# theblackcat102/edgedict

Hardware: AMD Instinct MI355X
Metric: utterances/sec (E6D2, 15 s audio) (higher is better)
Workload: dtype bf16; 1 GPU; E6D2 full training step (dither+log-mel+stack3+SpecAugment masks -> 6x1024 LSTM encoder, 2x time reduction -> 2x256 LSTM prediction net -> joint 640 -> RNN-T loss -> backward -> grad all-reduce -> Adam); 64 x 15 s utterances per GPU, U=64, V=2048, ragged lengths; lattice [64,201,65,2048]; global_batch=64, parallelism=dp1

## Files before the change

edgedict_amd/csrc/encoder_stack.hip:

```cpp
#include <stdio.h>
#include <stdlib.h>

#include <algorithm>
#include <mutex>
#include <vector>

#include "stack_kernels.hpp"

int ed_gemm_quiet_partials(int dtype_in, const void* A, long long lda, int a_kmajor, const void* B,
                           long long ldb, int b_kmajor, int M, int N, int K, int split_k,
                           int max_wg_per_cu, float* partials, int* slices, hipStream_t stream);

namespace {

__device__ __forceinline__ uint4 pack8(const float* v) {
    uint4 o;
    o.x = (unsigned)f32_to_bf16(v[0]) | ((unsigned)f32_to_bf16(v[1]) << 16);
    o.y = (unsigned)f32_to_bf16(v[2]) | ((unsigned)f32_to_bf16(v[3]) << 16);
    o.z = (unsigned)f32_to_bf16(v[4]) | ((unsigned)f32_to_bf16(v[5]) << 16);
    o.w = (unsigned)f32_to_bf16(v[6]) | ((unsigned)f32_to_bf16(v[7]) << 16);
    return o;
}
__device__ __forceinline__ int row_of_kap(int kap, int H) { return ((kap >> 4) & 3) * H + (kap >> 6) * 16 + (kap & 15); }

__global__ void pack_wih_kernel(const float* __restrict__ W, const float* __restrict__ b_ih,
                                const float* __restrict__ b_hh, bf16_t* __restrict__ Wp,
                                bf16_t* __restrict__ Wt, float* __restrict__ bp, int H, int I) {
    const long long n = 4ll * H * I;
    for (long long i = (long long)blockIdx.x * blockDim.x + threadIdx.x; i < n;
         i += (long long)gridDim.x * blockDim.x) {
        const int row = (int)(i / I), k = (int)(i % I);
        const int g = row / H, j = row % H;
        const int kap = ed_gate_col(g, j);
        const bf16_t v = f32_to_bf16(W[i]);
        Wp[(long long)kap * I + k] = v;
        if (Wt) Wt[(long long)k * 4 * H + kap] = v;
        if (k == 0) bp[kap] = b_ih[row] + b_hh[row];
    }
}
// ... 94 lines not shown
    for (long long c = (long long)blockIdx.x * blockDim.x + threadIdx.x; c < n4; c += (long long)gridDim.x * blockDim.x) {
        const int row = (int)(c / K4), k = (int)(c % K4) * 4;
        const long long o = (long long)ed_gate_col(row / H, row % H) * K + k;
        float4 v = make_float4(0.f, 0.f, 0.f, 0.f);
        for (int sl = 0; sl < S; ++sl) {
            const float4 p = *reinterpret_cast<const float4*>(src + sl * slice_stride + o);
            v.x += p.x; v.y += p.y; v.z += p.z; v.w += p.w;
        }
        const long long i = (long long)row * K + k;
        if (accumulate) {
            const float4 d = *reinterpret_cast<const float4*>(dst + i);
            *reinterpret_cast<float4*>(dst + i) = make_float4(d.x + v.x, d.y + v.y, d.z + v.z, d.w + v.w);
            if (dst2) {
                const float4 e = *reinterpret_cast<const float4*>(dst2 + i);
                *reinterpret_cast<float4*>(dst2 + i) = make_float4(e.x + v.x, e.y + v.y, e.z + v.z, e.w + v.w);
            }
        } else {
            *reinterpret_cast<float4*>(dst + i) = v;
            if (dst2) *reinterpret_cast<float4*>(dst2 + i) = v;
        }
    }
}
int unpermute_rows(const float* src, long long slice_stride, int S, float* dst, float* dst2, int H, int K, int accumulate,
                   hipStream_t s) {
    const bool vec = K % 4 == 0 && slice_stride % 4 == 0 && (uintptr_t)src % 16 == 0 && (uintptr_t)dst % 16 == 0 &&
                     (uintptr_t)dst2 % 16 == 0;
    if (vec)
        hipLaunchKernelGGL(unpermute_rows4_kernel, dim3(ed_grid_for(4ll * H * K / 4, 256, 4096)), dim3(256), 0, s, src,
                           slice_stride, S, dst, dst2, H, K, accumulate);
    else
        hipLaunchKernelGGL(unpermute_rows_kernel, dim3(ed_grid_for(4ll * H * K, 256, 4096)), dim3(256), 0, s, src,
                           slice_stride, S, dst, dst2, H, K, accumulate);
    ED_CHECK_LAUNCH("unpermute_rows_kernel");
    return ED_OK;
}

struct Runtime {
    std::mutex mu;
    hipStream_t R = nullptr, W = nullptr;
    int prio_hi = 0;
    hipEvent_t tev[2][2] = {{nullptr, nullptr}, {nullptr, nullptr}};
    int tlaunches[2] = {0, 0};
    int tkind[2] = {0, 0}, tsteps[2] = {0, 0};
    bool time_each = false;
    static constexpr int STAMP_SLOTS = 4096;
    unsigned long long* stamps[2] = {nullptr, nullptr};
    int stamp_used[2] = {0, 0};
    unsigned long long* stamp_slot(int i, hipStream_t s) {
        if (!time_each) return nullptr;
        if (!stamps[i] && hipMalloc((void**)&stamps[i], (size_t)STAMP_SLOTS * 16) != hipSuccess) {
            stamps[i] = nullptr;
            return nullptr;
        }
        if (stamp_used[i] == 0) {
            if (hipMemsetAsync(stamps[i], 0, (size_t)STAMP_SLOTS * 16, s) != hipSuccess) return nullptr;
            if (hipMemset2DAsync(stamps[i], 16, 0xff, 8, STAMP_SLOTS, s) != hipSuccess) return nullptr;
        }
        if (stamp_used[i] >= STAMP_SLOTS) return nullptr;
        return stamps[i] + 2 * (size_t)stamp_used[i]++;
    }
    unsigned* wsr_err_host = nullptr;
    unsigned* wsr_err_dev = nullptr;
    hipStream_t lazy(hipStream_t& s) {
        if (!s && hipStreamCreateWithPriority(&s, hipStreamNonBlocking, prio_hi) != hipSuccess) s = nullptr;
        return s;
    }
// ... 136 lines not shown
    for (int l = 0; l < d->L; ++l) {
        const edgedict_stack_layer_t& y = d->layers[l];
        ED_CHECK_ARG(y.T == T && y.I == I, "encoder_stack: layer %d geometry (T=%d I=%d) does not follow from the layers above (T=%d I=%d)", l, y.T, y.I, T, I);
        ED_CHECK_ARG(!y.residual || y.I == d->H, "encoder_stack: layer %d: residual needs I == H", l);
        ED_CHECK_ARG(y.drop_p >= 0.f && y.drop_p < 1.f, "encoder_stack: layer %d: dropout probability must be in [0, 1)", l);
        ED_CHECK_ARG(y.wih_p && y.bias_p && y.whh_f && y.ln_gamma && y.ln_beta && y.X && y.G && y.Yx && y.Cx && y.mean && y.rstd, "encoder_stack: layer %d: null pointer", l);
        if (backward)
            ED_CHECK_ARG(y.whh_b && y.dZ && (l == 0 || y.dX) && y.dW_ih && y.dW_hh && y.db && y.dgamma && y.dbeta, "encoder_stack: layer %d: null backward pointer", l);
        g[l].m = g[0].f / g[l].f;
        g[l].cf = d->chunk * g[l].f;
        g[l].nchunks = (y.T + g[l].cf - 1) / g[l].cf;
        T = (T + y.reduce - 1) / y.reduce;
        I = d->H;
    }
    ED_CHECK_ARG(d->ws_bytes >= ws_layout(d).total, "encoder_stack: workspace too small");
    return ED_OK;
}

struct Pace {
    static bool allows(int w, int l, int m_l, int m_min_running) {
        const int period = max(1, m_l / max(1, m_min_running));
        return period <= 1 || ((w + period * 1024 - (l % period)) % period) == 0;
    }
};

int margin_launches(const edgedict_stack_desc_t* d, const std::vector<Geom>& g, bool backward) {
    const int P = d->chunk * g[0].f;
    if (d->lag > 0) return max(1, d->lag - P + (backward ? 1 : 0));
    static const int mf = [] { const char* e = getenv("EDGEDICT_STACK_MARGIN_F"); return e ? atoi(e) : 0; }();
    static const int mb = [] { const char* e = getenv("EDGEDICT_STACK_MARGIN_B"); return e ? atoi(e) : 0; }();
    if (backward ? mb > 0 : mf > 0) return backward ? mb : mf;
    return backward ? 6 : 3;
}

#define ED_TRY(expr)            \
    do {                        \
        int st__ = (expr);      \
        if (st__ != ED_OK) return st__; \
    } while (0)

struct ScheduleTrace {
    int32_t* step_launch = nullptr;
    int32_t* chunk_enqueued = nullptr;
    std::vector<int> toff, coff;
    int launches = 0, max_slots = 0;
};
thread_local ScheduleTrace* g_trace = nullptr;
#define ED_DEV(expr)                      \
    do {                                  \
        if (!g_trace) ED_TRY(expr);       \
    } while (0)

struct Streams {
    hipStream_t C, R, R2, W;
    int split;
    int which(int l) const { return l >= split ? 1 : 0; }
    hipStream_t RS(int l) const { return which(l) ? R2 : R; }
    hipStream_t S[ED_STACK_MAX_SLOTS];
    bool serial;
    Runtime* rt;
    std::unique_lock<std::mutex> lock;
    hipEvent_t shared_ev = nullptr;
    hipStream_t shared_src = nullptr;
    int share(hipStream_t src) {
        if (serial) return ED_OK;
        shared_ev = rt->get();
        ED_CHECK_ARG(shared_ev != nullptr, "encoder_stack: event creation failed");
        ED_CHECK_HIP(hipEventRecord(shared_ev, src));
        shared_src = src;
        return ED_OK;
    }
    void unshare() { shared_ev = nullptr; shared_src = nullptr; }
// ... 717 lines not shown
                 "stack_launch_times: nothing recorded (edgedict_stack_time_launches(1) first)");
    const int n = r->stamp_used[i];
    std::vector<unsigned long long> h(2 * (size_t)n);
    ED_CHECK_HIP(hipStreamSynchronize(r->R));
    ED_CHECK_HIP(hipMemcpy(h.data(), r->stamps[i], h.size() * sizeof(unsigned long long), hipMemcpyDeviceToHost));
    double ticks = 0.0;
    int ok = 0;
    for (int k = 0; k < n; ++k)
        if (h[2 * k + 1] > h[2 * k]) {
            ticks += (double)(h[2 * k + 1] - h[2 * k]);
            ++ok;
        }
    ED_CHECK_ARG(ok > 0, "stack_launch_times: no launch stamped");
    *sum_ms = (float)(ticks * 1e-5);
    *launches = ok;
    return ED_OK;
}

extern "C" int edgedict_stack_launch_stamps(int backward, unsigned long long* out, int max_launches, int* launches) {
    ED_CHECK_ARG(out && launches && max_launches > 0, "stack_launch_stamps: bad arguments");
    Runtime* r = runtime_for_current_device();
    std::unique_lock<std::mutex> lock;
    if (r) lock = std::unique_lock<std::mutex>(r->mu);
    const int i = backward ? 1 : 0;
    ED_CHECK_ARG(r && r->stamps[i] && r->stamp_used[i] > 0,
                 "stack_launch_stamps: nothing recorded (edgedict_stack_time_launches(1) first)");
    const int n = min(max_launches, r->stamp_used[i]);
    ED_CHECK_HIP(hipDeviceSynchronize());
    ED_CHECK_HIP(hipMemcpy(out, r->stamps[i], (size_t)n * 16, hipMemcpyDeviceToHost));
    *launches = n;
    return ED_OK;
}

extern "C" int edgedict_stack_backward(const edgedict_stack_desc_t* d, void* stream_) {
    std::vector<Geom> g;
    ED_TRY(validate(d, g, true));
    ED_CHECK_ARG(d->dout && d->d_in_gamma && d->d_in_beta, "encoder_stack: null backward pointer in descriptor");
    ED_CHECK_ARG(!(d->flags & EDGEDICT_STACK_INFERENCE), "encoder_stack: backward on a descriptor flagged EDGEDICT_STACK_INFERENCE");
    const int B = d->B, H = d->H, L = d->L;
    const long long BH = (long long)B * H;
    const WsLayout wl = ws_layout(d);
    char* ws = (char*)d->ws;
    Streams st;
    ED_TRY(open_streams(d, stream_, st));
    st.R2 = st.R;
    st.split = L;
    const int T_out = (g[L - 1].T + d->layers[L - 1].reduce - 1) / d->layers[L - 1].reduce;

    static const int soft_env = [] { const char* e = getenv("EDGEDICT_STACK_SOFT_WAIT"); return e ? atoi(e) : 1; }();
    const bool soft = soft_env && !st.serial && L <= 8;
    unsigned* bflag = reinterpret_cast<unsigned*>(ws + wl.wsr_sync) + SYNC_BFLAG;
    unsigned* gerr = (st.rt && st.rt->wsr_err_dev) ? st.rt->wsr_err_dev + 2 : nullptr;
    if (soft)
        for (int l = 0; l < L; ++l) ED_CHECK_ARG(g[l].nchunks <= 512, "encoder_stack: too many chunks for the flag table");
    const int sk_ns = sk_bwd_steps(d);
    if (st.rt) {
        st.rt->tkind[1] = sk_ns ? 2 : 0;
        st.rt->tsteps[1] = sk_ns;
    }
    unsigned* cntb = reinterpret_cast<unsigned*>(ws + wl.wsr_sync) + SYNC_BCNT;
    unsigned* gcnt = reinterpret_cast<unsigned*>(ws + wl.wsr_sync) + SYNC_GCNT;
    if (sk_ns) {
        if (poison_on())
            for (int l = 0; l < L; ++l) {
                ED_DEV(ed_stack_fill(ws + wl.gimg[l], 0xff, (size_t)(d->layers[l].T + 1) * wl.gimg_stride, st.C));
                ED_DEV(ed_stack_fill(ws + wl.skpart[l], 0xff, (size_t)2 * (H / 64) * 4 * 64 * 64 * sizeof(float), st.C));
// ... 8 lines not shown
    ED_TRY(st.chain(st.C, st.W));

    std::vector<std::vector<hipEvent_t>> Eb(L);
    std::vector<std::vector<char>> queued(L);
    for (int l = 0; l < L; ++l) {
        Eb[l].assign(g[l].nchunks, nullptr);
        queued[l].assign(g[l].nchunks, l == L - 1 ? 1 : 0);
    }
    {
        const edgedict_stack_layer_t& y = d->layers[L - 1];
        hipStream_t S = st.S[L - 1];
        const DropCfg dcT = drop_of(y);
        for (int k = g[L - 1].nchunks - 1; k >= 0; --k) {
            const int t0 = k * g[L - 1].cf, t1 = min(y.T, t0 + g[L - 1].cf);
            ED_DEV(ed_stack_ln_bwd(bptr(d->dout), H, (long long)T_out * H, bptr(y.Yx) + BH,
                                   y.residual ? bptr(y.X) : nullptr, y.ln_gamma, y.mean, y.rstd, bptr(y.dZ),
                                   (float*)(ws + wl.lnpart[L - 1]) + (size_t)k * LNB_GRID * 2 * H, LNB_GRID, B, H,
                                   t0, t1, y.reduce, S, dcT.thresh, dcT.seed, dcT.scale, dcT.T_out));
            if (soft) ED_DEV(ed_stack_set_flag(bflag + (L - 1) * 512 + k, S));
            else ED_TRY(st.record(Eb[L - 1][k], S));
        }
    }
    std::vector<int> deferred;

    const int acc_grads = (d->flags & EDGEDICT_STACK_ACCUM_GRADS) ? 1 : 0;
    auto weight_grads = [&](int l, int t0, int t1, bool first, bool last_of_all) -> int {
        if (g_trace) {
            if (t0 == 0 && d->grads_final) d->grads_final(l, d->grads_final_user);
            return ED_OK;
        }
        const edgedict_stack_layer_t& y = d->layers[l];
        const int M = (t1 - t0) * B;
        const long long r0 = (long long)t0 * B;
        float* tmpW = (float*)(ws + wl.tmpW);
        float* tmpB = (float*)(ws + wl.tmpB);
        const int sk = d->split_k > 0 ? d->split_k : (last_of_all ? 8 : 2);
        const int cap = last_of_all ? 4 : 2;
        const int acc = (acc_grads || !first) ? 1 : 0;
        int S = 1;
        ED_TRY(ed_gemm_quiet_partials(ED_BF16, bptr(y.G) + r0 * 4 * H, 4ll * H, 0, bptr(y.X) + r0 * y.I, y.I, 0,
                                      4 * H, y.I, M, sk, cap, tmpW, &S, st.W));
        ED_TRY(unpermute_rows(tmpW, 4ll * H * y.I, S, y.dW_ih, nullptr, H, y.I, acc, st.W));
        ED_TRY(ed_gemm_quiet_partials(ED_BF16, bptr(y.G) + r0 * 4 * H, 4ll * H, 0, bptr(y.Yx) + r0 * H, H, 0,
                                      4 * H, H, M, sk, cap, tmpW, &S, st.W));
        ED_TRY(unpermute_rows(tmpW, 4ll * H * H, S, y.dW_hh, nullptr, H, H, acc, st.W));
        ED_TRY(ed_stack_zero(tmpB, (size_t)4 * H * sizeof(float), st.W));
        ED_TRY(edgedict_colsum(ED_BF16, bptr(y.G) + r0 * 4 * H, 4ll * H, tmpB, M, 4 * H, st.W));
        hipLaunchKernelGGL(unpermute_rows_kernel, dim3(ed_grid_for(4ll * H, 256, 4096)), dim3(256),
                           0, st.W, tmpB, 0, 1, y.db, y.db_hh, H, 1, acc);
        ED_CHECK_LAUNCH("unpermute_rows_kernel");
        if (t0 == 0 && d->grads_final) d->grads_final(l, d->grads_final_user);
        return ED_OK;
    };
    int dw_seg = 1 << 20;
    if (const char* e = getenv("EDGEDICT_STACK_DW_SEG")) dw_seg = max(1, atoi(e));
    if (d->flags & EDGEDICT_STACK_DW_AT_END) dw_seg = 1 << 20;
    int tail_split = 0;
    if (const char* e = getenv("EDGEDICT_STACK_TAIL_SPLIT")) tail_split = atoi(e);

    int margin = margin_launches(d, g, true);
    std::vector<int> next_t(L, 0);
    std::vector<std::vector<int>> ready_w(L);
    for (int l = 0; l < L; ++l) ready_w[l].assign(g[l].nchunks, l == L - 1 ? 0 : 0x3fffffff);
    auto after_recurrence = [&](int l, hipStream_t waiter) -> int { return st.chain(st.RS(l), waiter); };
    auto chunk_done = [&](int l, int k, int w) -> int {
            const edgedict_stack_layer_t& y = d->layers[l];
            if (l > 0) {
                const edgedict_stack_layer_t& z = d->layers[l - 1];
                const int t0 = k * g[l].cf, t1 = min(y.T, t0 + g[l].cf);
                const long long r0 = (long long)t0 * B;
                hipStream_t S = st.S[l];
                ED_TRY(after_recurrence(l, S));
                ED_DEV(edgedict_gemm(ED_BF16, ED_BF16, bptr(y.G) + r0 * 4 * H, 4ll * H, 1,
                                     y.wih_t ? y.wih_t : y.wih_p, y.wih_t ? 4ll * H : y.I,
                                     y.wih_t ? 1 : 0, bptr(y.dX) + r0 * y.I, y.I, (t1 - t0) * B, y.I,
                                     4 * H, nullptr, nullptr, y.dX == y.dZ ? 1 : 0, 1, S));
                const int u0 = k * g[l - 1].cf, u1 = min(z.T, u0 + g[l - 1].cf);
                ED_DEV(ed_stack_ln_bwd(bptr(y.dX), (long long)B * y.I, y.I, bptr(z.Yx) + BH,
                                       z.residual ? bptr(z.X) : nullptr, z.ln_gamma, z.mean, z.rstd,
                                       bptr(z.dZ), (float*)(ws + wl.lnpart[l - 1]) + (size_t)k * LNB_GRID * 2 * H,
                                       LNB_GRID, B, H, u0, u1, z.reduce, S, drop_of(z).thresh, drop_of(z).seed,
                                       drop_of(z).scale, drop_of(z).T_out));
                if (soft) ED_DEV(ed_stack_set_flag(bflag + (l - 1) * 512 + k, S));
                else ED_TRY(st.record(Eb[l - 1][k], S));
                queued[l - 1][k] = 1;
                ready_w[l - 1][k] = w + margin;
                if (g_trace) g_trace->chunk_enqueued[g_trace->coff[l - 1] + k] = g_trace->launches;
            }
            const int k_split = (l <= 1 && tail_split > 1 && g[l].nchunks >= 2 * tail_split && dw_seg >= g[l].nchunks &&
                                 !(d->flags & EDGEDICT_STACK_DW_AT_END))
                                    ? g[l].nchunks / tail_split : 0;
// ... 198 lines not shown
```

edgedict_amd/csrc/gemm_nt.hpp:

```cpp
#pragma once
#include <hip/hip_runtime.h>
bool ed_gemm_nt_ok(int dtype_in, int dtype_out, const void* A, long long lda, int a_kmajor,
                   const void* B, long long ldb, int b_kmajor, const void* C, long long ldc, int M,
                   int N, int K, int split_k, const float* bias1, const float* bias2);
int ed_gemm_nt_launch(const void* A, long long lda, const void* B, long long ldb, void* C,
                      long long ldc, int M, int N, int K, const float* bias1, const float* bias2,
                      int accumulate, int lds_pad, hipStream_t s);
bool ed_gemm_nt256_ok(int M, int N, int K, int accumulate);
bool ed_gemm_nt256_shape_ok(int M, int N, int K);
int ed_gemm_nt256_launch(const void* A, long long lda, const void* B, long long ldb, void* C,
                         long long ldc, int M, int N, int K, const float* bias1, const float* bias2,
                         hipStream_t s, float* lse_part = nullptr);
bool ed_gemm_nt256r_ok(int M, int N, int K, bool has_bias, int* grid_out = nullptr);
int ed_gemm_nt256r_launch(const void* A, long long lda, const void* B, long long ldb, void* C, long long ldc, int M,
                          int N, int K, const float* bias1, const float* bias2, hipStream_t s, float* lse_part);
bool ed_gemm_tn256_ok(const void* A, long long lda, const void* B, long long ldb, int M, int N, int K);
int ed_gemm_tn256_slices(int M, int N, int K, int max_slices);
int ed_gemm_tn256_partials(const void* A, long long lda, const void* B, long long ldb, float* partials, int M,
                           int N, int K, int slices, int max_wgs, hipStream_t s);
```

edgedict_amd/csrc/gemm_tn256.hip:

```cpp
#include <stdlib.h>

#include "common.hpp"
#include "gemm_nt.hpp"

namespace {

typedef __attribute__((ext_vector_type(8))) __bf16 bf16x8_t;
typedef __attribute__((ext_vector_type(4))) short s16x4_t;
typedef __attribute__((ext_vector_type(8))) short s16x8_t;
typedef __attribute__((ext_vector_type(4))) float f32x4_t;

constexpr int TM = 256, TN = 128, BK = 32;
constexpr int A_ST = BK * TM * 2;
constexpr int B_ST = BK * TN * 2;
constexpr int STAGE = A_ST + B_ST;
constexpr int NSTAGE = 4;
constexpr int LDS_BYTES = NSTAGE * STAGE;

__device__ uint4 g_zero_line[4];

struct Tn256Args {
    const bf16_t* A;
    const bf16_t* B;
    float* P;
    long long lda, ldb, pstride;
    int M, N, K;
    int n_tiles, tiles, slices, k_per, items, per;
};

__device__ __forceinline__ void glds16(const bf16_t* src, unsigned char* lds_wave_base) {
    __builtin_amdgcn_global_load_lds((const __attribute__((address_space(1))) void*)src,
                                     (__attribute__((address_space(3))) void*)lds_wave_base, 16, 0, 0);
}

__device__ __forceinline__ bf16x8_t tr_frag(const unsigned char* p0, const unsigned char* p1) {
    const s16x4_t lo = __builtin_amdgcn_ds_read_tr16_b64_v4i16((__attribute__((address_space(3))) s16x4_t*)p0);
    const s16x4_t hi = __builtin_amdgcn_ds_read_tr16_b64_v4i16((__attribute__((address_space(3))) s16x4_t*)p1);
    const s16x8_t v = __builtin_shufflevector(lo, hi, 0, 1, 2, 3, 4, 5, 6, 7);
    return __builtin_bit_cast(bf16x8_t, v);
}

__global__ __launch_bounds__(512, 2) void gemm_tn256_kernel(Tn256Args g) {
    extern __shared__ __attribute__((aligned(1024))) unsigned char smem[];
    const int lane = threadIdx.x & 63, wave = threadIdx.x >> 6;
    const int wm = wave >> 1, wn = wave & 1;
    const int r16 = lane & 15, kq = lane >> 4;

    const int krow = (wave & 3) * 8 + (lane >> 3);
    const int pw = wave >> 2;
    const int schunk = (lane & 7) ^ (lane >> 3);

    int tr_off[2];
#pragma unroll
    for (int h = 0; h < 2; ++h) {
        const int k = 16 * h + 4 * kq + (r16 >> 2);
        tr_off[h] = k * 128 + (((((r16 & 3) >> 1) ^ (k & 7))) << 4) + (r16 & 1) * 8;
    }

    const int G = gridDim.x, b = blockIdx.x;
    const int pos = (G % 8 == 0) ? (b % 8) * (G / 8) + b / 8 : b;
    const int item_end = min(g.items, (pos + 1) * g.per);
    for (int item = pos * g.per; item < item_end; ++item) {
        const int s = item / g.tiles, t = item % g.tiles;
        const int m0 = (t / g.n_tiles) * TM, n0 = (t % g.n_tiles) * TN;
        const int kbeg = s * g.k_per, kend = min(g.K, kbeg + g.k_per);
        const int NQ = (kend - kbeg + BK - 1) / BK;

        const bf16_t* asrc[2];
#pragma unroll
        for (int i = 0; i < 2; ++i) asrc[i] = g.A + min(m0 + (2 * i + pw) * 64 + schunk * 8, g.M - 8);
        const bf16_t* bsrc = g.B + min(n0 + pw * 64 + schunk * 8, g.N - 8);
        const bf16_t* zero = reinterpret_cast<const bf16_t*>(g_zero_line);

        auto issue = [&](int q) {
            unsigned char* base = smem + (q & (NSTAGE - 1)) * STAGE + (wave & 3) * 1024;
            const int k = kbeg + q * BK + krow;
            const bool in = k < kend;
            const long long ra = (long long)k * g.lda, rb = (long long)k * g.ldb;
#pragma unroll
            for (int i = 0; i < 2; ++i) glds16(in ? asrc[i] + ra : zero, base + (2 * i + pw) * 4096);
            glds16(in ? bsrc + rb : zero, base + A_ST + pw * 4096);
        };

        f32x4_t acc[4][4];
#pragma unroll
        for (int i = 0; i < 4; ++i)
#pragma unroll
            for (int j = 0; j < 4; ++j) acc[i][j] = (f32x4_t){0.f, 0.f, 0.f, 0.f};

        const int grp = wave >> 2;
        __syncthreads();
        issue(0);
        if (NQ > 1) issue(1);
        if (NQ > 2) issue(2);
        if (NQ > 2) asm volatile("s_waitcnt vmcnt(6)" ::: "memory");
        else if (NQ > 1) asm volatile("s_waitcnt vmcnt(3)" ::: "memory");
        else asm volatile("s_waitcnt vmcnt(0)" ::: "memory");
        asm volatile("s_barrier" ::: "memory");
        if (grp == 1) asm volatile("s_barrier" ::: "memory");
        for (int q = 0; q < NQ; ++q) {
            const unsigned char* sA = smem + (q & (NSTAGE - 1)) * STAGE + wm * 4096;
            const unsigned char* sB = smem + (q & (NSTAGE - 1)) * STAGE + A_ST + wn * 4096;
            bf16x8_t bf[4], af[4];
#pragma unroll
            for (int j = 0; j < 4; ++j)
                bf[j] = tr_frag(sB + (tr_off[0] ^ (j << 5)), sB + (tr_off[1] ^ (j << 5)));
#pragma unroll
            for (int i = 0; i < 4; ++i)
                af[i] = tr_frag(sA + (tr_off[0] ^ (i << 5)), sA + (tr_off[1] ^ (i << 5)));
            if (q + 3 < NQ) issue(q + 3);
            const int younger = min(NQ - 1, q + 3) - (q + 1);
            if (younger >= 2) asm volatile("s_waitcnt vmcnt(6)" ::: "memory");
            else if (younger == 1) asm volatile("s_waitcnt vmcnt(3)" ::: "memory");
            else asm volatile("s_waitcnt vmcnt(0)" ::: "memory");
            asm volatile("s_waitcnt lgkmcnt(0)" ::: "memory");
            asm volatile("s_barrier" ::: "memory");
            __builtin_amdgcn_s_setprio(1);
#pragma unroll
            for (int i = 0; i < 4; ++i)
#pragma unroll
                for (int j = 0; j < 4; ++j)
                    acc[i][j] = __builtin_amdgcn_mfma_f32_16x16x32_bf16(bf[j], af[i], acc[i][j], 0, 0, 0);
            __builtin_amdgcn_s_setprio(0);
            asm volatile("s_barrier" ::: "memory");
        }
        if (grp == 0) asm volatile("s_barrier" ::: "memory");
        float* P = g.P + (long long)s * g.pstride;
#pragma unroll
        for (int i = 0; i < 4; ++i) {
            const int row = m0 + wm * 64 + i * 16 + r16;
            if (row >= g.M) continue;
#pragma unroll
            for (int j = 0; j < 4; ++j) {
                const int col = n0 + wn * 64 + j * 16 + kq * 4;
                if (col >= g.N) continue;
                *reinterpret_cast<float4*>(P + (long long)row * g.N + col) =
                    make_float4(acc[i][j][0], acc[i][j][1], acc[i][j][2], acc[i][j][3]);
            }
        }
    }
}

}

bool ed_gemm_tn256_ok(const void* A, long long lda, const void* B, long long ldb, int M, int N, int K) {
    static const int on = [] { const char* e = getenv("EDGEDICT_GEMM_TN256"); return e ? atoi(e) : 1; }();
    return on && A && B && M >= 8 && N >= 8 && K >= 1 && M % 8 == 0 && N % 8 == 0 && lda % 8 == 0 && ldb % 8 == 0 &&
           (uintptr_t)A % 16 == 0 && (uintptr_t)B % 16 == 0;
}

int ed_gemm_tn256_slices(int M, int N, int K, int max_slices) {
    const long long tiles = (long long)((M + TM - 1) / TM) * ((N + TN - 1) / TN);
    int n_cu = 256, dev = 0;
    if (hipGetDevice(&dev) != hipSuccess ||
        hipDeviceGetAttribute(&n_cu, hipDeviceAttributeMultiprocessorCount, dev) != hipSuccess || n_cu <= 0)
        n_cu = 256;
    long long s = n_cu / (tiles > 0 ? tiles : 1);
    if (s > max_slices) s = max_slices;
    const int stages = (K + BK - 1) / BK;
    while (s > 1 && s * 8 > stages) --s;
    return s < 1 ? 1 : (int)s;
}

int ed_gemm_tn256_partials(const void* A, long long lda, const void* B, long long ldb, float* partials, int M,
                           int N, int K, int slices, int max_wgs, hipStream_t s) {
    ED_CHECK_ARG(partials && slices >= 1 && slices <= 64, "gemm_tn256: bad partials / slices");
    Tn256Args g;
    g.A = (const bf16_t*)A; g.B = (const bf16_t*)B; g.P = partials;
    g.lda = lda; g.ldb = ldb; g.pstride = (long long)M * N;
    g.M = M; g.N = N; g.K = K;
    g.n_tiles = (N + TN - 1) / TN;
    const long long tiles = (long long)((M + TM - 1) / TM) * g.n_tiles;
    ED_CHECK_ARG(tiles * slices < (1ll << 30), "gemm_tn256: too many tiles");
    g.tiles = (int)tiles;
    g.slices = slices;
    g.k_per = ((K + slices - 1) / slices + 63) / 64 * 64;
    g.items = g.tiles * slices;
    static const int n_cu = [] {
        int dev = 0, n = 256;
        if (hipGetDevice(&dev) != hipSuccess ||
            hipDeviceGetAttribute(&n, hipDeviceAttributeMultiprocessorCount, dev) != hipSuccess)
            n = 256;
        return n > 0 ? n : 256;
    }();
    int grid = n_cu;
    if (max_wgs > 0 && max_wgs < grid) grid = max_wgs;
    if (grid > g.items) grid = g.items;
    if (grid > 8) grid = grid / 8 * 8;
    g.per = (g.items + grid - 1) / grid;
    grid = (g.items + g.per - 1) / g.per;
    ED_CHECK_HIP(hipFuncSetAttribute((const void*)gemm_tn256_kernel,
                                     hipFuncAttributeMaxDynamicSharedMemorySize, LDS_BYTES));
    hipLaunchKernelGGL(gemm_tn256_kernel, dim3((unsigned)grid), dim3(512), LDS_BYTES, s, g);
    ED_CHECK_LAUNCH("gemm_tn256");
    return ED_OK;
}
```

include/edgedict_hip.h:

```cpp
#ifndef EDGEDICT_HIP_H
#define EDGEDICT_HIP_H

#include <stddef.h>
#include <stdint.h>

#ifdef __cplusplus
extern "C" {
#endif

#define EDGEDICT_ABI_VERSION 1

#define ED_OK 0
#define ED_ERR_INVALID (-1)
#define ED_ERR_LAUNCH (-2)

#define ED_F32 0
#define ED_BF16 1

const char* edgedict_last_error(void);
int edgedict_abi_version(void);

size_t edgedict_rnnt_workspace_bytes(int B, int T, int U1);
int edgedict_rnnt_loss_forward(const void* acts, int acts_dtype, const int32_t* labels,
                               const int32_t* act_lens, const int32_t* label_lens, int B, int T,
// ... 151 lines not shown
    const float* in_gamma;
    const float* in_beta;
    float* in_mean;
    float* in_rstd;
    const float* h0;
    const float* c0;
    void* out;
    const void* dout;
    float* d_in_gamma;
    float* d_in_beta;
    void* ws;
    size_t ws_bytes;
    void (*grads_final)(int layer, void* user);
    void* grads_final_user;
} edgedict_stack_desc_t;

size_t edgedict_stack_struct_bytes(int which);
void* edgedict_aux_stream(int which);
int edgedict_streams_busy(unsigned* mask);
size_t edgedict_stack_workspace_bytes(const edgedict_stack_desc_t* desc);
int edgedict_stack_pack_weights(const float* w_ih, const float* w_hh, const float* b_ih,
                                const float* b_hh, int H, int I, void* wih_p, void* wih_t,
                                float* bias_p, void* whh_f, void* whh_b, void* stream);
int edgedict_stack_pack_sk(const float* w_hh, int H, void* whh_s, void* stream);
int edgedict_stack_wsr_error(void);
void* edgedict_stack_error_words(int host);
int edgedict_stack_wsr_set_trace(void* device_buffer);
int edgedict_stack_forward(const edgedict_stack_desc_t* desc, void* stream);
int edgedict_stack_last_timing(int backward, float* ms, int* launches);
int edgedict_stack_last_mode(int backward, int* kind, int* steps_per_launch);
int edgedict_stack_time_launches(int on);
int edgedict_stack_launch_times(int backward, float* sum_ms, int* launches);
int edgedict_stack_launch_stamps(int backward, unsigned long long* out, int max_launches, int* launches);
int edgedict_stack_schedule(const edgedict_stack_desc_t* d, int backward, int32_t* step_launch,
                            int32_t* chunk_enqueued, int32_t* n_launches, int32_t* max_slots);
int edgedict_stack_backward(const edgedict_stack_desc_t* desc, void* stream);

int edgedict_cast(int src_dtype, const void* src, int dst_dtype, void* dst, long long n,
                  void* stream);
int edgedict_transpose(int src_dtype, const void* src, int dst_dtype, void* dst, int R, int C,
                       void* stream);
int edgedict_colsum(int dtype, const void* x, long long ld, float* out, long long M, int N,
                    void* stream);
int edgedict_embedding_fwd(int out_dtype, int emb_dtype, const int32_t* tokens, int tok_stride,
                           const void* emb, void* out, int B, int Uout, int E, int V,
                           int prepend_bos, int bos, void* stream);
int edgedict_embedding_bwd(int dtype, const int32_t* tokens, int tok_stride, const void* dout,
                           float* demb, int B, int Uout, int E, int V, int prepend_bos, int bos,
                           int pad, void* stream);
int edgedict_dropout(int dtype, const void* x, void* y, long long n, float p, unsigned seed,
                     void* stream);
int edgedict_spec_mask(float* x, int B, int T, int F, const int32_t* t_iv, int n_t,
                       const int32_t* f_iv, int n_f, void* stream);
int edgedict_joint_hidden_fwd(int dtype, const void* E1, const void* D1, void* hid, int B, int T,
                              int U1, int J, void* stream);
int edgedict_joint_hidden_bwd(int dtype, const void* dhid, const void* hid, float* dE1,
                              float* dD1, int B, int T, int U1, int J, void* stream);
int edgedict_joint_hidden_fwd_packed(int dtype, const void* E1, const void* D1, void* hid,
                                     const int32_t* act_lens, const int32_t* label_lens,
                                     const long long* row_offsets, int B, int T, int U1, int J,
                                     void* stream);
int edgedict_joint_hidden_bwd_packed(int dtype, const void* dhid, const void* hid, float* dE1,
                                     float* dD1, const int32_t* act_lens, const int32_t* label_lens,
                                     const long long* row_offsets, int B, int T, int U1, int J,
                                     void* stream);

// ... 202 lines not shown
```

Before: 3371 utterances/s.

## Fuse LSTM weight-gradient GEMMs and bias reduction into one stacked tn256 launch

Encoder backward weight gradients previously ran two split-K GEMMs into partials, each followed by an unpermute pass, plus a separate column-sum for the bias. They now go through a templated tn256 kernel that computes dW_ih and dW_hh tiles in one launch. It folds the bias sum into extra MFMA ops using a ones-vector trick and, when one slice suffices, writes permuted rows straight into the gradient buffers with optional accumulation. This removes launches and partial-buffer round trips, at the cost of extra per-tile branching, a bias MFMA on some waves, and launch bounds raised from 2 to 4 waves per EU, which may squeeze registers.

Result: no change. 3395 utterances/s, median of 6 (+0.7%).

```diff
diff --git a/edgedict_amd/csrc/encoder_stack.hip b/edgedict_amd/csrc/encoder_stack.hip
--- a/edgedict_amd/csrc/encoder_stack.hip
+++ b/edgedict_amd/csrc/encoder_stack.hip
@@ -5,6 +5,7 @@
 #include <mutex>
 #include <vector>
 
+#include "gemm_nt.hpp"
 #include "stack_kernels.hpp"
 
 int ed_gemm_quiet_partials(int dtype_in, const void* A, long long lda, int a_kmajor, const void* B,
@@ -165,6 +166,81 @@
         hipLaunchKernelGGL(unpermute_rows_kernel, dim3(ed_grid_for(4ll * H * K, 256, 4096)), dim3(256), 0, s, src,
                            slice_stride, S, dst, dst2, H, K, accumulate);
     ED_CHECK_LAUNCH("unpermute_rows_kernel");
+    return ED_OK;
+}
+
+#define ED_TRY(expr)            \
+    do {                        \
+        int st__ = (expr);      \
+        if (st__ != ED_OK) return st__; \
+    } while (0)
+
+int stack_weight_grads(const bf16_t* dG, long long ldg, const bf16_t* X, long long ldx, int I, const bf16_t* Hp,
+                       long long ldh, int H, int rows, float* dW_ih, float* dW_hh, float* db, float* db_hh,
+                       int acc, float* scratch, long long scratch_floats, float* tmpB, int sk, int cap, bool thresholds,
+                       int slices_override, int* route, hipStream_t s) {
+    static const int merge_env = [] { const char* e = getenv("EDGEDICT_STACK_DW_MERGE"); return e ? atoi(e) : 1; }();
+    static const int bias_env = [] { const char* e = getenv("EDGEDICT_STACK_DW_BIAS"); return e ? atoi(e) : 1; }();
+    static const int fuse_env = [] { const char* e = getenv("EDGEDICT_STACK_DW_FUSE"); return e ? atoi(e) : 1; }();
+    const int M = 4 * H;
+    const bool big = !thresholds || ((long long)M * I >= (1ll << 18) && (long long)M * H >= (1ll << 18) && rows >= 1024);
+    const bool fast = fuse_env && big && H % 16 == 0 && ed_gemm_tn256_ok(dG, ldg, X, ldx, M, I, rows) &&
+                      ed_gemm_tn256_ok(dG, ldg, Hp, ldh, M, H, rows) && (uintptr_t)dW_ih % 16 == 0 &&
+                      (uintptr_t)dW_hh % 16 == 0;
+    if (!fast) {
+        if (route) *route = EDGEDICT_DW_FALLBACK;
+        int S = 1;
+        ED_CHECK_ARG(scratch_floats >= 8ll * M * max(I, H), "stack_weight_grads: scratch too small");
+        ED_TRY(ed_gemm_quiet_partials(ED_BF16, dG, ldg, 0, X, ldx, 0, M, I, rows, sk, cap, scratch, &S, s));
+        ED_TRY(unpermute_rows(scratch, (long long)M * I, S, dW_ih, nullptr, H, I, acc, s));
+        ED_TRY(ed_gemm_quiet_partials(ED_BF16, dG, ldg, 0, Hp, ldh, 0, M, H, rows, sk, cap, scratch, &S, s));
+        ED_TRY(unpermute_rows(scratch, (long long)M * H, S, dW_hh, nullptr, H, H, acc, s));
+    }
+    bool bias_done = false;
+    if (fast) {
+        const bool merged = merge_env >= 2 || (merge_env == 1 && ed_gemm_tn256_stack_tiles(M, I, H) <= ed_gemm_tn256_cus());
+        const bool fb = bias_env != 0;
+        bias_done = fb;
+        auto product = [&](const bf16_t* B0, long long ld0, int N0, float* out0, const bf16_t* B1, long long ld1, int N1,
+                           float* out1, bool with_bias, int* S_out) -> int {
+            const long long per = (long long)M * (N0 + (B1 ? N1 : 0) + (with_bias ? 1 : 0));
+            int S = slices_override > 0 ? slices_override
+                                        : (B1 ? ed_gemm_tn256_stack_slices(M, N0, N1, rows, 8)
+                                              : ed_gemm_tn256_slices(M, N0, rows, 8));
+            if (slices_override <= 0)
+                while (S > 1 && S * per > scratch_floats) --S;
+            ED_CHECK_ARG(S == 1 || S * per <= scratch_floats, "stack_weight_grads: %d slices do not fit the scratch", S);
+            *S_out = S;
+            if (S == 1)
+                return ed_gemm_tn256_stack(dG, ldg, B0, ld0, N0, B1, ld1, N1, H, rows, out0, out1, with_bias ? db : nullptr,
+                                           with_bias ? db_hh : nullptr, acc, 1, s);
+            float* p0 = scratch;
+            float* p1 = p0 + (long long)S * M * N0;
+            float* pb = p1 + (B1 ? (long long)S * M * N1 : 0);
+            ED_TRY(ed_gemm_tn256_stack(dG, ldg, B0, ld0, N0, B1, ld1, N1, H, rows, p0, p1, with_bias ? pb : nullptr, nullptr,
+                                       0, S, s));
+            ED_TRY(unpermute_rows(p0, (long long)M * N0, S, out0, nullptr, H, N0, acc, s));
+            if (B1) ED_TRY(unpermute_rows(p1, (long long)M * N1, S, out1, nullptr, H, N1, acc, s));
+            if (with_bias) ED_TRY(unpermute_rows(pb, M, S, db, db_hh, H, 1, acc, s));
+            return ED_OK;
+        };
+        int S0 = 1, S1 = 1;
+        if (merged) {
+            ED_TRY(product(X, ldx, I, dW_ih, Hp, ldh, H, dW_hh, fb, &S0));
+            if (route) *route = S0 == 1 ? EDGEDICT_DW_FUSED_DIRECT : EDGEDICT_DW_FUSED_PARTIALS;
+        } else {
+            ED_TRY(product(X, ldx, I, dW_ih, nullptr, 0, 0, nullptr, fb, &S0));
+            ED_TRY(product(Hp, ldh, H, dW_hh, nullptr, 0, 0, nullptr, false, &S1));
+            if (route) *route = EDGEDICT_DW_TWO_LAUNCH;
+        }
+    }
+    if (!bias_done) {
+        ED_TRY(ed_stack_zero(tmpB, (size_t)M * sizeof(float), s));
+        ED_TRY(edgedict_colsum(ED_BF16, dG, ldg, tmpB, rows, M, s));
+        hipLaunchKernelGGL(unpermute_rows_kernel, dim3(ed_grid_for((long long)M, 256, 4096)), dim3(256), 0, s, tmpB, 0, 1,
+                           db, db_hh, H, 1, acc);
+        ED_CHECK_LAUNCH("unpermute_rows_kernel");
+    }
     return ED_OK;
 }
 
@@ -367,12 +443,6 @@
     if (backward ? mb > 0 : mf > 0) return backward ? mb : mf;
     return backward ? 6 : 3;
 }
-
-#define ED_TRY(expr)            \
-    do {                        \
-        int st__ = (expr);      \
-        if (st__ != ED_OK) return st__; \
-    } while (0)
 
 struct ScheduleTrace {
     int32_t* step_launch = nullptr;
@@ -1156,6 +1226,24 @@
     return ED_OK;
 }
 
+extern "C" int edgedict_stack_weight_grads(const void* dG, long long ldg, const void* X, long long ldx, int I,
+                                           const void* Hprev, int H, int rows, float* dW_ih, float* dW_hh, float* db,
+                                           float* db_hh, int accumulate, int slices_override, float* scratch,
+                                           long long scratch_floats, int* route_out, void* stream_) {
+    ED_CHECK_ARG(dG && X && Hprev && dW_ih && dW_hh && db && db_hh && scratch && route_out,
+                 "stack_weight_grads: null pointer");
+    ED_CHECK_ARG(I >= 1 && H >= 16 && H % 16 == 0 && rows >= 1 && ldg >= 4ll * H && ldx >= I,
+                 "stack_weight_grads: bad shape (I=%d H=%d rows=%d)", I, H, rows);
+    ED_CHECK_ARG(slices_override >= 0 && slices_override <= 8, "stack_weight_grads: slices_override must be 0..8");
+    ED_CHECK_ARG(scratch_floats >= 8ll * 4 * H * max(I, H) + 4ll * H,
+                 "stack_weight_grads: scratch must hold 8 * 4H * max(I, H) + 4H floats");
+    *route_out = -1;
+    const long long tmpW_floats = scratch_floats - 4ll * H;
+    return stack_weight_grads((const bf16_t*)dG, ldg, (const bf16_t*)X, ldx, I, (const bf16_t*)Hprev, H, H, rows, dW_ih,
+                              dW_hh, db, db_hh, accumulate ? 1 : 0, scratch, tmpW_floats, scratch + tmpW_floats, 2, 2,
+                              false, slices_override, route_out, (hipStream_t)stream_);
+}
+
 extern "C" int edgedict_stack_backward(const edgedict_stack_desc_t* d, void* stream_) {
     std::vector<Geom> g;
     ED_TRY(validate(d, g, true));
@@ -1230,31 +1318,21 @@
         const edgedict_stack_layer_t& y = d->layers[l];
         const int M = (t1 - t0) * B;
         const long long r0 = (long long)t0 * B;
-        float* tmpW = (float*)(ws + wl.tmpW);
-        float* tmpB = (float*)(ws + wl.tmpB);
         const int sk = d->split_k > 0 ? d->split_k : (last_of_all ? 8 : 2);
         const int cap = last_of_all ? 4 : 2;
         const int acc = (acc_grads || !first) ? 1 : 0;
-        int S = 1;
-        ED_TRY(ed_gemm_quiet_partials(ED_BF16, bptr(y.G) + r0 * 4 * H, 4ll * H, 0, bptr(y.X) + r0 * y.I, y.I, 0,
-                                      4 * H, y.I, M, sk, cap, tmpW, &S, st.W));
-        ED_TRY(unpermute_rows(tmpW, 4ll * H * y.I, S, y.dW_ih, nullptr, H, y.I, acc, st.W));
-        ED_TRY(ed_gemm_quiet_partials(ED_BF16, bptr(y.G) + r0 * 4 * H, 4ll * H, 0, bptr(y.Yx) + r0 * H, H, 0,
-                                      4 * H, H, M, sk, cap, tmpW, &S, st.W));
-        ED_TRY(unpermute_rows(tmpW, 4ll * H * H, S, y.dW_hh, nullptr, H, H, acc, st.W));
-        ED_TRY(ed_stack_zero(tmpB, (size_t)4 * H * sizeof(float), st.W));
-        ED_TRY(edgedict_colsum(ED_BF16, bptr(y.G) + r0 * 4 * H, 4ll * H, tmpB, M, 4 * H, st.W));
-        hipLaunchKernelGGL(unpermute_rows_kernel, dim3(ed_grid_for(4ll * H, 256, 4096)), dim3(256),
-                           0, st.W, tmpB, 0, 1, y.db, y.db_hh, H, 1, acc);
-        ED_CHECK_LAUNCH("unpermute_rows_kernel");
+        ED_TRY(stack_weight_grads(bptr(y.G) + r0 * 4 * H, 4ll * H, bptr(y.X) + r0 * y.I, y.I, y.I, bptr(y.Yx) + r0 * H, H, H,
+                                  M, y.dW_ih, y.dW_hh, y.db, y.db_hh, acc, (float*)(ws + wl.tmpW),
+                                  (long long)(wl.tmpB - wl.tmpW) / (long long)sizeof(float), (float*)(ws + wl.tmpB), sk, cap,
+                                  true, 0, nullptr, st.W));
         if (t0 == 0 && d->grads_final) d->grads_final(l, d->grads_final_user);
         return ED_OK;
     };
-    int dw_seg = 1 << 20;
-    if (const char* e = getenv("EDGEDICT_STACK_DW_SEG")) dw_seg = max(1, atoi(e));
+    static const int dw_seg_env = [] { const char* e = getenv("EDGEDICT_STACK_DW_SEG"); return e ? max(1, atoi(e)) : 1 << 20; }();
+    static const int tail_split_env = [] { const char* e = getenv("EDGEDICT_STACK_TAIL_SPLIT"); return e ? atoi(e) : 0; }();
+    int dw_seg = dw_seg_env;
     if (d->flags & EDGEDICT_STACK_DW_AT_END) dw_seg = 1 << 20;
-    int tail_split = 0;
-    if (const char* e = getenv("EDGEDICT_STACK_TAIL_SPLIT")) tail_split = atoi(e);
+    const int tail_split = tail_split_env;
 
     int margin = margin_launches(d, g, true);
     std::vector<int> next_t(L, 0);
diff --git a/edgedict_amd/csrc/gemm_nt.hpp b/edgedict_amd/csrc/gemm_nt.hpp
--- a/edgedict_amd/csrc/gemm_nt.hpp
+++ b/edgedict_amd/csrc/gemm_nt.hpp
@@ -18,3 +18,9 @@
 int ed_gemm_tn256_slices(int M, int N, int K, int max_slices);
 int ed_gemm_tn256_partials(const void* A, long long lda, const void* B, long long ldb, float* partials, int M,
                            int N, int K, int slices, int max_wgs, hipStream_t s);
+int ed_gemm_tn256_stack_tiles(int M, int N0, int N1);
+int ed_gemm_tn256_stack_slices(int M, int N0, int N1, int K, int max_slices);
+int ed_gemm_tn256_cus();
+int ed_gemm_tn256_stack(const void* A, long long lda, const void* B0, long long ldb0, int N0, const void* B1,
+                        long long ldb1, int N1, int H, int K, float* out0, float* out1, float* bias0, float* bias1,
+                        int accumulate, int slices, hipStream_t s);
diff --git a/edgedict_amd/csrc/gemm_tn256.hip b/edgedict_amd/csrc/gemm_tn256.hip
--- a/edgedict_amd/csrc/gemm_tn256.hip
+++ b/edgedict_amd/csrc/gemm_tn256.hip
@@ -9,6 +9,7 @@
 typedef __attribute__((ext_vector_type(4))) short s16x4_t;
 typedef __attribute__((ext_vector_type(8))) short s16x8_t;
 typedef __attribute__((ext_vector_type(4))) float f32x4_t;
+typedef __attribute__((ext_vector_type(4))) int s32x4_t;
 
 constexpr int TM = 256, TN = 128, BK = 32;
 constexpr int A_ST = BK * TM * 2;
@@ -26,6 +27,12 @@
     long long lda, ldb, pstride;
     int M, N, K;
     int n_tiles, tiles, slices, k_per, items, per;
+    const bf16_t* B1;
+    float* P1;
+    float* bias0;
+    float* bias1;
+    long long ldb1, pstride1;
+    int N1, n_tiles0, H, direct, accumulate;
 };
 
 __device__ __forceinline__ void glds16(const bf16_t* src, unsigned char* lds_wave_base) {
@@ -40,7 +47,8 @@
     return __builtin_bit_cast(bf16x8_t, v);
 }
 
-__global__ __launch_bounds__(512, 2) void gemm_tn256_kernel(Tn256Args g) {
+template <bool STACK>
+__global__ __launch_bounds__(512, 4) void gemm_tn256_kernel(Tn256Args g) {
     extern __shared__ __attribute__((aligned(1024))) unsigned char smem[];
     const int lane = threadIdx.x & 63, wave = threadIdx.x >> 6;
     const int wm = wave >> 1, wn = wave & 1;
@@ -62,21 +70,29 @@
     const int item_end = min(g.items, (pos + 1) * g.per);
     for (int item = pos * g.per; item < item_end; ++item) {
         const int s = item / g.tiles, t = item % g.tiles;
-        const int m0 = (t / g.n_tiles) * TM, n0 = (t % g.n_tiles) * TN;
+        const int m0 = (t / g.n_tiles) * TM;
+        int nt = t % g.n_tiles;
+        const bool op1 = STACK && nt >= g.n_tiles0;
+        if (op1) nt -= g.n_tiles0;
+        const int n0 = nt * TN;
+        const bf16_t* Bop = op1 ? g.B1 : g.B;
+        const long long ldb = op1 ? g.ldb1 : g.ldb;
+        const int N = op1 ? g.N1 : g.N;
+        const bool bias = STACK && g.bias0 && !op1 && nt == 0 && wn == 0;
         const int kbeg = s * g.k_per, kend = min(g.K, kbeg + g.k_per);
         const int NQ = (kend - kbeg + BK - 1) / BK;
 
         const bf16_t* asrc[2];
 #pragma unroll
         for (int i = 0; i < 2; ++i) asrc[i] = g.A + min(m0 + (2 * i + pw) * 64 + schunk * 8, g.M - 8);
-        const bf16_t* bsrc = g.B + min(n0 + pw * 64 + schunk * 8, g.N - 8);
+        const bf16_t* bsrc = Bop + min(n0 + pw * 64 + schunk * 8, N - 8);
         const bf16_t* zero = reinterpret_cast<const bf16_t*>(g_zero_line);
 
         auto issue = [&](int q) {
             unsigned char* base = smem + (q & (NSTAGE - 1)) * STAGE + (wave & 3) * 1024;
             const int k = kbeg + q * BK + krow;
             const bool in = k < kend;
-            const long long ra = (long long)k * g.lda, rb = (long long)k * g.ldb;
+            const long long ra = (long long)k * g.lda, rb = (long long)k * ldb;
 #pragma unroll
             for (int i = 0; i < 2; ++i) glds16(in ? asrc[i] + ra : zero, base + (2 * i + pw) * 4096);
             glds16(in ? bsrc + rb : zero, base + A_ST + pw * 4096);
@@ -87,6 +103,7 @@
         for (int i = 0; i < 4; ++i)
 #pragma unroll
             for (int j = 0; j < 4; ++j) acc[i][j] = (f32x4_t){0.f, 0.f, 0.f, 0.f};
+        f32x4_t bacc = (f32x4_t){0.f, 0.f, 0.f, 0.f};
 
         const int grp = wave >> 2;
         __syncthreads();
@@ -121,21 +138,52 @@
 #pragma unroll
                 for (int j = 0; j < 4; ++j)
                     acc[i][j] = __builtin_amdgcn_mfma_f32_16x16x32_bf16(bf[j], af[i], acc[i][j], 0, 0, 0);
+            if (STACK && bias) {
+#pragma unroll
+                for (int i = 0; i < 4; ++i) {
+                    int sel = r16;
+                    asm volatile("" : "+v"(sel));
+                    const int w = (sel >> 2) == i ? 0x3f803f80 : 0;
+                    bacc = __builtin_amdgcn_mfma_f32_16x16x32_bf16(__builtin_bit_cast(bf16x8_t, (s32x4_t){w, w, w, w}), af[i],
+                                                                   bacc, 0, 0, 0);
+                }
+            }
             __builtin_amdgcn_s_setprio(0);
             asm volatile("s_barrier" ::: "memory");
         }
         if (grp == 0) asm volatile("s_barrier" ::: "memory");
-        float* P = g.P + (long long)s * g.pstride;
+        const bool direct = STACK && g.direct;
+        float* P = op1 ? g.P1 : g.P;
+        if (!direct) P += (long long)s * (op1 ? g.pstride1 : g.pstride);
 #pragma unroll
         for (int i = 0; i < 4; ++i) {
             const int row = m0 + wm * 64 + i * 16 + r16;
             if (row >= g.M) continue;
+            const int orow = direct ? ((row >> 4) & 3) * g.H + (row >> 6) * 16 + (row & 15) : row;
 #pragma unroll
             for (int j = 0; j < 4; ++j) {
                 const int col = n0 + wn * 64 + j * 16 + kq * 4;
-                if (col >= g.N) continue;
-                *reinterpret_cast<float4*>(P + (long long)row * g.N + col) =
-                    make_float4(acc[i][j][0], acc[i][j][1], acc[i][j][2], acc[i][j][3]);
+                if (col >= N) continue;
+                float4* dst = reinterpret_cast<float4*>(P + (long long)orow * N + col);
+                float4 v = make_float4(acc[i][j][0], acc[i][j][1], acc[i][j][2], acc[i][j][3]);
+                if (direct && g.accumulate) {
+                    const float4 d = *dst;
+                    v.x += d.x; v.y += d.y; v.z += d.z; v.w += d.w;
+                }
+                *dst = v;
+            }
+        }
+        if (STACK && bias) {
+            const int row = m0 + wm * 64 + kq * 16 + r16;
+            if (row < g.M) {
+                const float v = bacc[0];
+                if (direct) {
+                    const int orow = ((row >> 4) & 3) * g.H + (row >> 6) * 16 + (row & 15);
+                    g.bias0[orow] = g.accumulate ? g.bias0[orow] + v : v;
+                    g.bias1[orow] = g.accumulate ? g.bias1[orow] + v : v;
+                } else {
+                    g.bias0[(long long)s * g.M + row] = v;
+                }
             }
         }
     }
@@ -149,33 +197,8 @@
            (uintptr_t)A % 16 == 0 && (uintptr_t)B % 16 == 0;
 }
 
-int ed_gemm_tn256_slices(int M, int N, int K, int max_slices) {
-    const long long tiles = (long long)((M + TM - 1) / TM) * ((N + TN - 1) / TN);
-    int n_cu = 256, dev = 0;
-    if (hipGetDevice(&dev) != hipSuccess ||
-        hipDeviceGetAttribute(&n_cu, hipDeviceAttributeMultiprocessorCount, dev) != hipSuccess || n_cu <= 0)
-        n_cu = 256;
-    long long s = n_cu / (tiles > 0 ? tiles : 1);
-    if (s > max_slices) s = max_slices;
-    const int stages = (K + BK - 1) / BK;
-    while (s > 1 && s * 8 > stages) --s;
-    return s < 1 ? 1 : (int)s;
-}
-
-int ed_gemm_tn256_partials(const void* A, long long lda, const void* B, long long ldb, float* partials, int M,
-                           int N, int K, int slices, int max_wgs, hipStream_t s) {
-    ED_CHECK_ARG(partials && slices >= 1 && slices <= 64, "gemm_tn256: bad partials / slices");
-    Tn256Args g;
-    g.A = (const bf16_t*)A; g.B = (const bf16_t*)B; g.P = partials;
-    g.lda = lda; g.ldb = ldb; g.pstride = (long long)M * N;
-    g.M = M; g.N = N; g.K = K;
-    g.n_tiles = (N + TN - 1) / TN;
-    const long long tiles = (long long)((M + TM - 1) / TM) * g.n_tiles;
-    ED_CHECK_ARG(tiles * slices < (1ll << 30), "gemm_tn256: too many tiles");
-    g.tiles = (int)tiles;
-    g.slices = slices;
-    g.k_per = ((K + slices - 1) / slices + 63) / 64 * 64;
-    g.items = g.tiles * slices;
+namespace {
+int tn256_cus() {
     static const int n_cu = [] {
         int dev = 0, n = 256;
         if (hipGetDevice(&dev) != hipSuccess ||
@@ -183,15 +206,78 @@
             n = 256;
         return n > 0 ? n : 256;
     }();
-    int grid = n_cu;
+    return n_cu;
+}
+int slices_for_tiles(long long tiles, int K, int max_slices) {
+    long long s = tn256_cus() / (tiles > 0 ? tiles : 1);
+    if (s > max_slices) s = max_slices;
+    const int stages = (K + BK - 1) / BK;
+    while (s > 1 && s * 8 > stages) --s;
+    return s < 1 ? 1 : (int)s;
+}
+template <bool STACK>
+int tn256_launch(Tn256Args& g, int slices, int max_wgs, hipStream_t s) {
+    const long long tiles = (long long)((g.M + TM - 1) / TM) * g.n_tiles;
+    ED_CHECK_ARG(tiles * slices < (1ll << 30), "gemm_tn256: too many tiles");
+    g.tiles = (int)tiles;
+    g.slices = slices;
+    g.k_per = ((g.K + slices - 1) / slices + 63) / 64 * 64;
+    g.items = g.tiles * slices;
+    int grid = tn256_cus();
     if (max_wgs > 0 && max_wgs < grid) grid = max_wgs;
     if (grid > g.items) grid = g.items;
     if (grid > 8) grid = grid / 8 * 8;
     g.per = (g.items + grid - 1) / grid;
     grid = (g.items + g.per - 1) / g.per;
-    ED_CHECK_HIP(hipFuncSetAttribute((const void*)gemm_tn256_kernel,
+    ED_CHECK_HIP(hipFuncSetAttribute((const void*)gemm_tn256_kernel<STACK>,
                                      hipFuncAttributeMaxDynamicSharedMemorySize, LDS_BYTES));
-    hipLaunchKernelGGL(gemm_tn256_kernel, dim3((unsigned)grid), dim3(512), LDS_BYTES, s, g);
+    hipLaunchKernelGGL(gemm_tn256_kernel<STACK>, dim3((unsigned)grid), dim3(512), LDS_BYTES, s, g);
     ED_CHECK_LAUNCH("gemm_tn256");
     return ED_OK;
 }
+}
+
+int ed_gemm_tn256_slices(int M, int N, int K, int max_slices) {
+    return slices_for_tiles((long long)((M + TM - 1) / TM) * ((N + TN - 1) / TN), K, max_slices);
+}
+
+int ed_gemm_tn256_stack_tiles(int M, int N0, int N1) {
+    return ((M + TM - 1) / TM) * ((N0 + TN - 1) / TN + (N1 + TN - 1) / TN);
+}
+int ed_gemm_tn256_stack_slices(int M, int N0, int N1, int K, int max_slices) {
+    return slices_for_tiles(ed_gemm_tn256_stack_tiles(M, N0, N1), K, max_slices);
+}
+int ed_gemm_tn256_cus() { return tn256_cus(); }
+
+int ed_gemm_tn256_partials(const void* A, long long lda, const void* B, long long ldb, float* partials, int M,
+                           int N, int K, int slices, int max_wgs, hipStream_t s) {
+    ED_CHECK_ARG(partials && slices >= 1 && slices <= 64, "gemm_tn256: bad partials / slices");
+    Tn256Args g = {};
+    g.A = (const bf16_t*)A; g.B = (const bf16_t*)B; g.P = partials;
+    g.lda = lda; g.ldb = ldb; g.pstride = (long long)M * N;
+    g.M = M; g.N = N; g.K = K;
+    g.n_tiles = (N + TN - 1) / TN;
+    return tn256_launch<false>(g, slices, max_wgs, s);
+}
+
+int ed_gemm_tn256_stack(const void* A, long long lda, const void* B0, long long ldb0, int N0, const void* B1,
+                        long long ldb1, int N1, int H, int K, float* out0, float* out1, float* bias0, float* bias1,
+                        int accumulate, int slices, hipStream_t s) {
+    const int M = 4 * H;
+    ED_CHECK_ARG(slices >= 1 && slices <= 64 && H > 0 && H % 16 == 0, "gemm_tn256_stack: bad slices / H");
+    ED_CHECK_ARG(ed_gemm_tn256_ok(A, lda, B0, ldb0, M, N0, K) && (!B1 || ed_gemm_tn256_ok(A, lda, B1, ldb1, M, N1, K)),
+                 "gemm_tn256_stack: operands must be 16-byte aligned with sizes and leading dimensions %% 8 == 0");
+    ED_CHECK_ARG(out0 && (uintptr_t)out0 % 16 == 0 && (!B1 || (out1 && (uintptr_t)out1 % 16 == 0)) &&
+                 (!bias0 || slices > 1 || bias1), "gemm_tn256_stack: bad output pointer");
+    Tn256Args g = {};
+    g.A = (const bf16_t*)A; g.lda = lda;
+    g.B = (const bf16_t*)B0; g.ldb = ldb0; g.N = N0; g.P = out0; g.pstride = (long long)M * N0;
+    g.B1 = (const bf16_t*)B1; g.ldb1 = ldb1; g.N1 = B1 ? N1 : 0; g.P1 = out1; g.pstride1 = (long long)M * N1;
+    g.bias0 = bias0; g.bias1 = bias1;
+    g.M = M; g.K = K; g.H = H;
+    g.direct = slices == 1 ? 1 : 0;
+    g.accumulate = accumulate;
+    g.n_tiles0 = (N0 + TN - 1) / TN;
+    g.n_tiles = g.n_tiles0 + (g.N1 + TN - 1) / TN;
+    return tn256_launch<true>(g, slices, 0, s);
+}
diff --git a/include/edgedict_hip.h b/include/edgedict_hip.h
--- a/include/edgedict_hip.h
+++ b/include/edgedict_hip.h
@@ -207,6 +207,14 @@
 int edgedict_stack_time_launches(int on);
 int edgedict_stack_launch_times(int backward, float* sum_ms, int* launches);
 int edgedict_stack_launch_stamps(int backward, unsigned long long* out, int max_launches, int* launches);
+#define EDGEDICT_DW_FALLBACK 0
+#define EDGEDICT_DW_FUSED_DIRECT 1
+#define EDGEDICT_DW_FUSED_PARTIALS 2
+#define EDGEDICT_DW_TWO_LAUNCH 3
+int edgedict_stack_weight_grads(const void* dG, long long ldg, const void* X, long long ldx, int I,
+                                const void* Hprev, int H, int rows, float* dW_ih, float* dW_hh, float* db,
+                                float* db_hh, int accumulate, int slices_override, float* scratch,
+                                long long scratch_floats, int* route_out, void* stream);
 int edgedict_stack_schedule(const edgedict_stack_desc_t* d, int backward, int32_t* step_launch,
                             int32_t* chunk_enqueued, int32_t* n_launches, int32_t* max_slots);
 int edgedict_stack_backward(const edgedict_stack_desc_t* desc, void* stream);
```
